# ace19-dev/gvcnn-tf

Measured on AMD Instinct MI355X. Metric: views/sec, higher is better.
Workload: dtype f32; 1 GPU; BASELINE.json configs[1]: ModelNet-shaped, 12 views x 224x224x3, inception_v3 backbone (raw tap Mixed_6e, final tap Mixed_7c), num_groups=7, f32, forward only; views_per_gpu=384, global_views=384, num_groups=7, num_classes=10, exchange=none, branch_lanes=3, launch=eager

## Files before the change

### gvcnn-tf_amd/build.py

```python
import os
import subprocess
import sys

HERE = os.path.dirname(os.path.abspath(__file__))
ROOT = os.path.dirname(HERE)
CSRC = os.path.join(HERE, "csrc")
PT = os.environ.get("GV_PHASE_TIMES") == "1"
LIB = os.path.join(HERE, "libgvcnn_hip_pt.so" if PT else "libgvcnn_hip.so")
BUILD = "build_pt" if PT else "build"
SOURCES = ["conv_igemm.hip", "conv_bf16s.hip", "conv_lp.hip", "conv_dma.hip", "conv_ws.hip", "conv_ws_x3.hip", "conv_chain.hip", "pool.hip", "lowp.hip", "grouping.hip", "plan.hip", "train.hip", "train_lp.hip", "wgrad_dma.hip",
           "retrieval.hip", "render.hip", "metric.hip", "scorer_bwd.hip", "png.hip", "explain.hip"]
FLAGS = ["--offload-arch=gfx950", "-O3", "-std=c++17", "-fPIC", "-Wall",
         "-I" + os.path.join(ROOT, "include"), "-I" + CSRC] + (["-DGV_PHASE_TIMES"] if PT else [])


def _stale(target, deps):
    if not os.path.exists(target):
        return True
    t = os.path.getmtime(target)
    return any(os.path.getmtime(d) > t for d in deps)


def build(force=False, verbose=False):
    hipcc = os.environ.get("HIPCC", "/opt/rocm/bin/hipcc")
    headers = [os.path.join(ROOT, "include", "gvcnn_hip.h")] + sorted(
        os.path.join(CSRC, f) for f in os.listdir(CSRC) if f.endswith(".h"))
    objs = []
    procs = []
    os.makedirs(os.path.join(HERE, BUILD), exist_ok=True)
    for s in SOURCES:
        src = os.path.join(CSRC, s)
        obj = os.path.join(HERE, BUILD, s.replace(".hip", ".o"))
        objs.append(obj)
        if force or _stale(obj, [src] + headers):
            cmd = [hipcc] + FLAGS + ["-c", src, "-o", obj]
            if verbose:
                print(" ".join(cmd))
            procs.append((cmd, subprocess.Popen(cmd)))
    for cmd, p in procs:
        if p.wait() != 0:
            raise RuntimeError("hipcc failed: " + " ".join(cmd))
    if force or procs or _stale(LIB, objs):
        cmd = [hipcc, "--offload-arch=gfx950", "-shared", "-fPIC", "-o", LIB] + objs
        if verbose:
            print(" ".join(cmd))
        subprocess.check_call(cmd)
    return LIB


if __name__ == "__main__":
    print(build(force="--force" in sys.argv, verbose=True))
```

### gvcnn-tf_amd/csrc/conv_common.h

```cpp
#pragma once
#include <cstdlib>

#include "gv_common.h"
#include "conv_stats.h"

namespace gvconv {

struct ConvArgs {
    const float* x;
    const void* w;
    const float* scale;
    const float* shift;
    const float* res;
    float* y;
    float* y2;
    const float* scale2;
    const float* shift2;
    int nb, ih, iw, cin, x_ld;
    int kh, kw, stride, pad_t, pad_l;
    int oh, ow, cout, y_ld, res_ld, y2_ld;
    int M, K, Kpad, ktiles;
    int relu, relu2, split;
    int relu_limit;
    int tiles_n;
    int dil_shift;
#ifdef GV_PHASE_TIMES
    unsigned long long* phase_buf = nullptr;
#endif
    int dbg;
    const void* zeros;
    int y_p3, y2_p3;
    int korder;
    const float* xscale;
    const float* xshift;
    ConvStats st;
    int y_step = 0;
    int y_py = 0, y_px = 0;
    int y_ih = 0, y_iw = 0;
    GvFastDiv y_div_img = {0, -1, 1}, y_div_row = {0, -1, 1};
    int pool = 0;
    int ph = 0, pw = 0;
};

inline bool lp_epilogue_lean_ok(const ConvArgs& a) {
    const bool one = a.y2 == nullptr && a.split == 0;
    const bool two = a.y2 != nullptr && a.split > 0 && a.split % 8 == 0 && a.y2_ld % 8 == 0 && (((uintptr_t)a.y2) & 15) == 0 &&
                     !a.y2_p3;
    return !(a.dbg & 2) && (one || two) && a.cout % 8 == 0 && a.y_ld % 8 == 0 &&
           (((uintptr_t)a.y) & 15) == 0 && (a.res == nullptr || (a.res_ld % 8 == 0 && (((uintptr_t)a.res) & 15) == 0)) &&
           (!a.relu || a.relu_limit >= a.cout || a.relu_limit % 8 == 0);
}

template <int TM, int TN>
__device__ __forceinline__ void conv_epilogue(const ConvArgs& a, const f32x16 (&acc)[TM][TN], int m0,
                                              int n0, int wm, int wn, int lane) {
    if (a.dbg & 4) {
        float t = 0.f;
#pragma unroll
        for (int i = 0; i < TM; ++i)
#pragma unroll
            for (int j = 0; j < TN; ++j)
#pragma unroll
                for (int r = 0; r < 16; ++r) t += acc[i][j][r];
        if (t == 1.2345e-30f) a.y[0] = t;
        return;
    }
    const int col_l = lane & 31;
    const int row_h = 4 * (lane >> 5);
#pragma unroll
    for (int j = 0; j < TN; ++j) {
        const int col = n0 + (wn * TN + j) * 32 + col_l;
        if (col >= a.cout) continue;
        const float sc = a.scale[col], sh = a.shift[col];
        const bool to_second = a.split > 0 && col >= a.split;
        const bool dual = a.y2 != nullptr && a.split == 0;
        const bool relu = a.relu && col < a.relu_limit;
        float sc2 = 0.f, sh2 = 0.f;
        if (dual) { sc2 = a.scale2[col]; sh2 = a.shift2[col]; }
        float* ybase = to_second ? a.y2 + (col - a.split) : a.y + col;
        const int yld = to_second ? a.y2_ld : a.y_ld;
#pragma unroll
        for (int i = 0; i < TM; ++i) {
            const int rbase = m0 + (wm * TM + i) * 32 + row_h;
#pragma unroll
            for (int r = 0; r < 16; ++r) {
                const int m = rbase + (r & 3) + 8 * (r >> 2);
                if (m >= a.M) continue;
                float v = acc[i][j][r] * sc + sh;
                if (a.res) v += a.res[(size_t)m * a.res_ld + col];
                if (dual) {
                    float v2 = v * sc2 + sh2;
                    if (a.relu2) v2 = fmaxf(v2, 0.f);
                    a.y2[(size_t)m * a.y2_ld + col] = v2;
                }
                if (relu) v = fmaxf(v, 0.f);
                ybase[(size_t)m * yld] = v;
            }
        }
    }
}

inline int64_t conv_grid(ConvArgs& a, int bm, int bn) {
    a.tiles_n = gv_ceil_div(a.cout, bn);
    const int64_t nwg = (int64_t)gv_ceil_div(a.M, bm) * a.tiles_n;
    return nwg > 0x7fffffff ? -1 : nwg;
}

inline bool ws_disabled() {
    static const bool off = getenv("GV_NO_WS") != nullptr;
    return off;
}

inline int staged_pick_tile(int M, int N) {
    int best = 0, best_bn = 128;
    double best_cost = 1e30;
    const int order[] = {0, 3, 1, 5}, bns[] = {128, 96, 64, 32};
    const double pen[] = {1.00, 1.02, 1.05, 1.20};
    for (int t = 0; t < 4; ++t) {
        const double cost = (double)gv_ceil_div(N, bns[t]) * bns[t] * pen[t];
        if (cost < best_cost) { best_cost = cost; best = order[t]; best_bn = bns[t]; }
    }
    const int64_t blocks = (int64_t)gv_ceil_div(M, 128) * gv_ceil_div(N, best_bn);
    if (blocks < 1024) {
        if (best_bn == 128) best = 4;
        else if (best_bn == 64) best = 2;
    }
    return best;
}


int bf16s_staged_num_cfgs();
int bf16s_staged_launch(int planes, int cfg, const ConvArgs& a, bool generic, hipStream_t st);
int bf16s_special_launch(int planes, const ConvArgs& a, bool generic, hipStream_t st);
bool bf16s_halo_ok(int planes, const ConvArgs& a, bool generic);
bool bf16s_stem_ok(int planes, const ConvArgs& a);
int bf16s_pack_filter(const float* w_hwio, int kh, int kw, int cin, int cout, int planes, void* out,
                      hipStream_t st);
int64_t bf16s_packed_bytes(int kh, int kw, int cin, int cout, int planes);

int lp_staged_num_cfgs();
int lp_staged_launch(int dtype, int cfg, const ConvArgs& a, bool generic, bool xf32, hipStream_t st);
int lp_special_launch(int dtype, const ConvArgs& a, bool generic, bool xf32, hipStream_t st);
bool lp_xpre_cfg_ok(int cfg);
int lp_xpre_pick(int M, int N);
bool lp_halo_ok(const ConvArgs& a, bool generic);
bool lp_stem_ok(const ConvArgs& a, bool xf32);
int lp_pack_filter(const float* w_hwio, int kh, int kw, int cin, int cout, int dtype, void* out, hipStream_t st);
int64_t lp_packed_bytes(int kh, int kw, int cin, int cout);
int lp_pack_filters_batched(const gv_pack_job* jobs_dev, const int* block_job_dev, int nblocks, int dtype, hipStream_t st);

int dma_lp_num_cfgs();
bool dma_lp_ok(const ConvArgs& a, bool generic, bool xf32);
int dma_lp_launch(int dtype, int cfg, const ConvArgs& a, hipStream_t st);
const void* dma_zero_page();
int dma_x3_num_cfgs();
bool dma_x3_ok(const ConvArgs& a);
int dma_x3_launch(int cfg, const ConvArgs& a, hipStream_t st);
bool chain_tail_ok(const ConvArgs& a);
int chain_tail_launch(int dtype, const ConvArgs& a, hipStream_t st);
int ws_lp_num_cfgs();
int ws_lp_launch(int dtype, int cfg, const ConvArgs& a, hipStream_t st);
int ws_x3_num_cfgs();
int ws_x3_launch(int cfg, const ConvArgs& a, hipStream_t st);
int wsg_x3_num_cfgs();
int wsg_x3_launch(int cfg, const ConvArgs& a, hipStream_t st);

}
```

### gvcnn-tf_amd/csrc/conv_ws_x3.hip

```cpp
#include <cstdlib>
#include <type_traits>

#include "conv_common.h"
#include "conv_lp_epi.h"
#include "conv_x3_epi.h"

namespace {

constexpr int X3W_HEAD = 64;
constexpr int X3W_NL = 4;

struct WsX3Args {
    int taps, nchunks, nk;
    int halo_lo;
    int strip_blocks;
    int pad_[3];
};

__device__ __forceinline__ void x3w_dma16(const char* gsrc, char* lds_dst) {
    __builtin_amdgcn_global_load_lds((const __attribute__((address_space(1))) void*)gsrc,
                                     (__attribute__((address_space(3))) void*)lds_dst, 16, 0, 0);
}
template <int N>
__device__ __forceinline__ void x3w_wait_vm() {
    static_assert(N >= 0 && N < 64, "vmcnt is a 6-bit counter");
    asm volatile("s_waitcnt vmcnt(%0)" ::"n"(N) : "memory");
}

__device__ __forceinline__ void x3w_gload16(f32x4& dst, const char* p) {
    asm volatile("global_load_dwordx4 %0, %1, off" : "=v"(dst) : "v"(p) : "memory");
}
template <int N>
__device__ __forceinline__ void x3w_wait_vm_reg(f32x4& r) {
    static_assert(N >= 0 && N < 64, "vmcnt is a 6-bit counter");
    asm volatile("s_waitcnt vmcnt(%1)" : "+v"(r) : "n"(N) : "memory");
}

template <int WM, int WN, int TM, int TN, int NB, int SBMAX, int GEMM = 0>
__global__ __launch_bounds__((WM * WN + X3W_NL) * 64, 3) void conv_ws_x3(const ConvArgs a, const WsX3Args w) {
    constexpr int NC = WM * WN;
    constexpr int BM = WM * TM * 32, BN = WN * TN * 32;
    constexpr int B_PLANE = BN * 32, B_SLOT = 3 * B_PLANE;
    constexpr int A_PLANE = GEMM ? BM * 32 : X3W_HEAD + SBMAX * 1024, S_BUF = 3 * A_PLANE;
    constexpr int NA = GEMM ? 3 : 2;
    constexpr int OFF_S = NB * B_SLOT;
    constexpr int UB3 = 3 * (BN / 32);
    constexpr int LB = (UB3 + X3W_NL - 1) / X3W_NL;
    static_assert(NC == 8, "eight consumer waves + four loaders: three waves per SIMD");
    static_assert(TM <= TN && TM * TN >= 4, "plane-2 fragments of a and b share one register block");
    static_assert(NB >= 3 && (NB - 1) * LB < 64, "ring depth / vmcnt range");
    static_assert(GEMM == 0 || (NB == 4 && BM % (16 * X3W_NL) == 0), "GEMM mode: four filter slots, 16-row load instructions");
    (void)NA;

    extern __shared__ __attribute__((aligned(128))) char smem[];
    const int tid = threadIdx.x;
    const int lane = tid & 63;
    const int wave = __builtin_amdgcn_readfirstlane(tid >> 6);
    const int lid = gv_xcd_remap(blockIdx.x, gridDim.x);
    const int tile_n = lid % a.tiles_n, tile_m = lid / a.tiles_n;
    const int m0 = tile_m * BM, n0 = tile_n * BN;
    const int nk = w.nk, NTAP = w.taps;
    const bool nosync = (a.dbg & (16384 | 65536)) != 0;

    static_assert(BN <= X3W_NL * 64, "one loader thread per tile column");
    float ss_v[2] = {0.f, 0.f};
    f32x16 acc[TM][TN];

    if (wave >= NC) {
        const int lw = wave - NC;
        if (tid - NC * 64 < BN) {
            const int cc = min(n0 + tid - NC * 64, a.cout - 1);
            ss_v[0] = a.scale[cc];
            ss_v[1] = a.shift[cc];
        }
        if (!(a.dbg & 16384)) {
            __builtin_amdgcn_s_setprio(3);
            const bool nodma = (a.dbg & 32768) != 0, nobar = (a.dbg & 65536) != 0;
            const int lrow = lane >> 1;
            const int lc16 = (((lane & 1) ^ ((lrow >> 3) & 1)) << 4);
            const char* xb = reinterpret_cast<const char*>(a.x);
            const char* b_ptr[LB];
            int b_dst[LB];
            {
                const size_t wrow = (size_t)(a.Kpad / 16) * 96;
#pragma unroll
                for (int i = 0; i < LB; ++i) {
                    int d = lw + i * X3W_NL;
                    d = d < UB3 ? d : UB3 - 1;
                    const int rb = d / 3, p = d - rb * 3;
                    int n = n0 + rb * 32 + lrow;
                    n = n < a.cout ? n : a.cout - 1;
                    b_ptr[i] = reinterpret_cast<const char*>(a.w) + (size_t)n * wrow + p * 32 + lc16;
                    b_dst[i] = p * B_PLANE + rb * 1024;
                }
            }
            int bq_t = 0, bq_c = 0, bq_slot = 0;
            const int gtap = (a.cin >> 4) * 96;
            auto issue_b = [&]() {
                const unsigned koff = (unsigned)(bq_t * gtap + bq_c * 96);
                char* sb = smem + bq_slot * B_SLOT;
#pragma unroll
                for (int i = 0; i < LB; ++i)
                    if (!nodma) x3w_dma16(b_ptr[i] + koff, sb + b_dst[i]);
                if (++bq_t == NTAP) { bq_t = 0; ++bq_c; }
                bq_slot = bq_slot + 1 == NB ? 0 : bq_slot + 1;
            };
            if constexpr (GEMM != 0) {
                constexpr int RPW = BM / X3W_NL, NI = RPW / 16;
                const int qd = lane & 3;
                const char* a_ptr[NI];
                int a_dst[NI];
#pragma unroll
                for (int i = 0; i < NI; ++i) {
                    const int row = lw * RPW + i * 16 + (lane >> 2);
                    int m = m0 + row;
                    m = m < a.M ? m : a.M - 1;
                    a_ptr[i] = xb + (size_t)(unsigned)m * ((size_t)a.x_ld * 4) + qd * 16;
                    a_dst[i] = OFF_S + row * 32 + ((((qd >> 1) ^ ((row >> 3) & 1))) << 4) + (qd & 1) * 8;
                }
                f32x4 stg[2][NI];
                auto load_a = [&](auto sc, int c) {
                    constexpr int S = decltype(sc)::value;
                    c = c < nk ? c : nk - 1;
#pragma unroll
                    for (int i = 0; i < NI; ++i) x3w_gload16(stg[S][i], a_ptr[i] + (size_t)c * 64);
                };
                auto wait_a = [&](auto sc, auto nc) {
                    constexpr int S = decltype(sc)::value;
                    constexpr int N = decltype(nc)::value;
#pragma unroll
                    for (int i = 0; i < NI; ++i) x3w_wait_vm_reg<N>(stg[S][i]);
                };
                auto write_a = [&](auto sc, int slot) {
                    constexpr int S = decltype(sc)::value;
                    char* sb = smem + slot * S_BUF;
#pragma unroll
                    for (int i = 0; i < NI; ++i) {
                        float v[4] = {stg[S][i][0], stg[S][i][1], stg[S][i][2], stg[S][i][3]};
#pragma unroll
                        for (int p = 0; p < 3; ++p) {
                            const unsigned lo = pack2<__bf16>(v[0], v[1]), hi = pack2<__bf16>(v[2], v[3]);
                            typedef unsigned u32x2_t __attribute__((ext_vector_type(2)));
                            *reinterpret_cast<u32x2_t*>(sb + p * A_PLANE + a_dst[i]) = u32x2_t{lo, hi};
                            if (p < 2) {
                                v[0] -= __builtin_bit_cast(float, lo << 16);
                                v[1] -= __builtin_bit_cast(float, lo & 0xffff0000u);
                                v[2] -= __builtin_bit_cast(float, hi << 16);
                                v[3] -= __builtin_bit_cast(float, hi & 0xffff0000u);
                            }
                        }
                    }
                };
                using S0 = std::integral_constant<int, 0>;
                using S1 = std::integral_constant<int, 1>;
                auto fetch = [&](auto sc, int k) {
                    issue_b();
                    load_a(sc, k);
                };
                fetch(S0{}, 0);
                fetch(S1{}, 1);
                wait_a(S0{}, std::integral_constant<int, 0>{});
                wait_a(S1{}, std::integral_constant<int, 0>{});
                write_a(S0{}, 0);
                write_a(S1{}, 1);
                fetch(S0{}, 2);
                fetch(S1{}, 3);
                asm volatile("s_waitcnt lgkmcnt(0)" ::: "memory");
                if (!nobar) __builtin_amdgcn_s_barrier();
                auto iter = [&](auto sc, int j) {
                    wait_a(sc, std::integral_constant<int, LB + NI>{});
                    if (j + 2 < nk) {
                        int slot = j + 2;
                        slot -= (slot / 3) * 3;
                        write_a(sc, slot);
                        asm volatile("s_waitcnt lgkmcnt(0)" ::: "memory");
                    }
                    if (!nobar) __builtin_amdgcn_s_barrier();
                    if (j + 4 >= nk) {
                        bq_c = nk - 1;
                        bq_slot = (nk - 1) & 3;
                    }
                    fetch(sc, j + 4);
                };
                for (int j = 0; j + 1 < nk; j += 2) {
                    iter(S0{}, j);
                    if (j + 2 < nk) iter(S1{}, j + 1);
                }
                x3w_wait_vm<0>();
            } else {
            const unsigned pix_bytes = (unsigned)a.x_ld * 6u;
            int sq_c = 0, sq_buf = 0;
            int sp_blk = 1 << 30, sp_p = 0, sp_c = 0, sp_buf = 0;
            auto strip_begin = [&]() {
                sp_blk = lw / 3; sp_p = lw - sp_blk * 3; sp_c = sq_c; sp_buf = sq_buf;
                ++sq_c;
                sq_buf ^= 1;
            };
            auto strip_units = [&](int n) {
                char* sb = smem + OFF_S + sp_buf * S_BUF + X3W_HEAD;
                const unsigned coff = (unsigned)sp_c * 96u + (unsigned)lc16;
                for (int i = 0; i < n && sp_blk < w.strip_blocks; ++i) {
                    int p = m0 - w.halo_lo + sp_blk * 32 + lrow;
                    p = p < 0 ? 0 : (p < a.M ? p : a.M - 1);
                    if (!nodma) x3w_dma16(xb + (size_t)(unsigned)p * pix_bytes + coff + sp_p * 32, sb + sp_p * A_PLANE + sp_blk * 1024);
                    ++sp_p; ++sp_blk;
                    if (sp_p == 3) { sp_p = 0; ++sp_blk; }
                }
            };
            const int upl = (3 * w.strip_blocks + X3W_NL - 1) / X3W_NL;
            const int win = max(NTAP - NB + 2, 1);
            const int ppi = (upl + win - 1) / win;
            strip_begin();
            strip_units(1 << 20);
            issue_b();
#pragma unroll
            for (int q = 1; q < NB; ++q) issue_b();
            x3w_wait_vm<(NB - 2) * LB>();
            if (!nobar) __builtin_amdgcn_s_barrier();
            if (w.nchunks > 1) { strip_begin(); strip_units(ppi); }
            int ft = 0;
            for (int j = 0; j + 1 < nk; ++j) {
                if (j + NB - 1 <= nk - 1) x3w_wait_vm<(NB - 3) * LB>();
                else x3w_wait_vm<0>();
                if (!nobar) __builtin_amdgcn_s_barrier();
                const bool last_tap = ft + 1 == NTAP;
                if (last_tap && sq_c < w.nchunks) strip_begin();
                strip_units(ppi);
                if (j + NB < nk) issue_b();
                ft = last_tap ? 0 : ft + 1;
            }
            x3w_wait_vm<0>();
            }
        }
    } else {
        const int wm = wave / WN, wn = wave % WN;
        const int r = lane & 31, h = lane >> 5;
        if constexpr (GEMM == 0) {
            if (tid < 96) {
                const int img = tid >> 4;
                *reinterpret_cast<unsigned*>(smem + OFF_S + (img / 3) * S_BUF + (img % 3) * A_PLANE + (tid & 15) * 4) = 0u;
            }
        }
#pragma unroll
        for (int i = 0; i < TM; ++i)
#pragma unroll
            for (int j = 0; j < TN; ++j)
#pragma unroll
                for (int q = 0; q < 16; ++q) acc[i][j][q] = 0.f;
        const int rbase0 = wm * TM * 32 + r + w.halo_lo;
        unsigned tapmask[TM];
        if constexpr (GEMM != 0) {
#pragma unroll
            for (int i = 0; i < TM; ++i) tapmask[i] = 0u;
        } else {
            const int ohow = a.oh * a.ow;
#pragma unroll
            for (int i = 0; i < TM; ++i) {
                const int lr = (wm * TM + i) * 32 + r;
                int m = m0 + lr;
                m = m < a.M ? m : a.M - 1;
                const int n = gv_div(m, a.y_div_img);
                const int rem = m - n * ohow;
                const int y = gv_div(rem, a.y_div_row);
                const int x = rem - y * a.ow;
                const int r_lo = max(0, a.pad_t - y), r_hi = min(a.kh, a.ih + a.pad_t - y);
                const int c_lo = max(0, a.pad_l - x), c_hi = min(a.kw, a.iw + a.pad_l - x);
                const unsigned rowbits = c_hi > c_lo ? (1u << c_hi) - (1u << c_lo) : 0u;
                unsigned tm = 0u;
                for (int fr = 0; fr < a.kh; ++fr)
                    if (fr >= r_lo && fr < r_hi) tm |= rowbits << (fr * a.kw);
                tapmask[i] = tm;
            }
        }
        const int h16 = h << 4;
        const int b_lane = (wn * TN * 32 + r) * 32 + ((((r >> 3) & 1) << 4) ^ h16);
        auto a_addr = [&](int i, int off, int tap, int sbase) -> int {
            if constexpr (GEMM != 0) return sbase + ((wm * TM + i) * 32 + r) * 32 + ((((r >> 3) & 1) << 4) ^ h16);
            const int row = rbase0 + i * 32 + off;
            const int ad = sbase + X3W_HEAD + row * 32 + ((((row >> 3) & 1) << 4) ^ h16);
            const int in = -(int)((tapmask[i] >> tap) & 1u);
            return (ad & in) | ((sbase + h16) & ~in);
        };
        auto lds16 = [&](int addr) -> u32x4 { return *reinterpret_cast<const u32x4*>(smem + addr); };
        u32x4 A0[TM], A1[TM], B0[TN], B1[TN], T[TN];
#define X3W_PIN() __builtin_amdgcn_sched_barrier(0)
        auto kstep = [&](auto nextc, int (&aa)[TM], int& bn, bool bar, auto&& next_addr) {
            constexpr bool NEXT = decltype(nextc)::value;
            constexpr int NM = TM * TN;
            X3W_PIN();
#pragma unroll
            for (int m = 0; m < NM; ++m) {
                const int i = m / TN, j = m % TN;
                acc[i][j] = mfma16<__bf16>(A0[i], T[j], acc[i][j]);
                if (i == TM - 1 && j < TM) { T[j] = lds16(aa[j] + 2 * A_PLANE); X3W_PIN(); }
            }
            X3W_PIN();
            next_addr();
#pragma unroll
            for (int m = 0; m < NM; ++m) {
                const int i = m / TN, j = m % TN;
                acc[i][j] = mfma16<__bf16>(A0[i], B1[j], acc[i][j]);
            }
            X3W_PIN();
#pragma unroll
            for (int m = 0; m < NM; ++m) {
                const int i = m / TN, j = m % TN;
                acc[i][j] = mfma16<__bf16>(A0[i], B0[j], acc[i][j]);
                if constexpr (NEXT) {
                    if (i == 0 && j >= TM && j < TN) { T[j] = lds16(bn + j * 1024 + 2 * B_PLANE); X3W_PIN(); }
                    if (j == TN - 1) { A0[i] = lds16(aa[i]); X3W_PIN(); }
                }
            }
            X3W_PIN();
#pragma unroll
            for (int m = 0; m < NM; ++m) {
                const int i = m / TN, j = m % TN;
                acc[i][j] = mfma16<__bf16>(T[i], B0[j], acc[i][j]);
                if constexpr (NEXT) {
                    if (j == TN - 1) { T[i] = lds16(bn + i * 1024 + 2 * B_PLANE); X3W_PIN(); }
                }
            }
            X3W_PIN();
#pragma unroll
            for (int m = 0; m < NM; ++m) {
                const int i = m / TN, j = m % TN;
                acc[i][j] = mfma16<__bf16>(A1[i], B0[j], acc[i][j]);
                if constexpr (NEXT) {
                    if (i == TM - 1) { B0[j] = lds16(bn + j * 1024); X3W_PIN(); }
                }
            }
            X3W_PIN();
#pragma unroll
            for (int m = 0; m < NM; ++m) {
                const int i = m / TN, j = m % TN;
                acc[i][j] = mfma16<__bf16>(A1[i], B1[j], acc[i][j]);
                if constexpr (NEXT) {
                    if (m == 1) {
                        X3W_PIN();
                        if (bar) __builtin_amdgcn_s_barrier();
                        X3W_PIN();
                    }
                    if (j == TN - 1) { A1[i] = lds16(aa[i] + A_PLANE); X3W_PIN(); }
                    if (i == TM - 1) { B1[j] = lds16(bn + j * 1024 + B_PLANE); X3W_PIN(); }
                }
            }
            X3W_PIN();
        };
        int q_fr = 0, q_fs = 0, q_tap = 0;
        int sbuf = 0, bslot = 0;
        int aa[TM];
#pragma unroll
        for (int i = 0; i < TM; ++i) aa[i] = a_addr(i, -(a.pad_t * a.iw + a.pad_l), 0, OFF_S);
        asm volatile("s_waitcnt lgkmcnt(0)" ::: "memory");
        if (!nosync) __builtin_amdgcn_s_barrier();
#pragma unroll
        for (int i = 0; i < TM; ++i) { A0[i] = lds16(aa[i]); A1[i] = lds16(aa[i] + A_PLANE); }
#pragma unroll
        for (int j = 0; j < TN; ++j) {
            B0[j] = lds16(b_lane + j * 1024);
            B1[j] = lds16(b_lane + j * 1024 + B_PLANE);
            T[j] = lds16(b_lane + j * 1024 + 2 * B_PLANE);
        }
        int bn = 0;
        auto next_addr = [&]() {
            if constexpr (GEMM != 0) {
                sbuf = sbuf + 1 == NA ? 0 : sbuf + 1;
#pragma unroll
                for (int i = 0; i < TM; ++i) aa[i] = a_addr(i, 0, 0, OFF_S + sbuf * S_BUF);
                bslot = bslot + B_SLOT == NB * B_SLOT ? 0 : bslot + B_SLOT;
                bn = b_lane + bslot;
                return;
            }
            const bool wrap = q_tap + 1 == NTAP;
            const bool row_end = q_fs + 1 == a.kw;
            q_tap = wrap ? 0 : q_tap + 1;
            q_fr = wrap ? 0 : (row_end ? q_fr + 1 : q_fr);
            q_fs = (wrap || row_end) ? 0 : q_fs + 1;
            sbuf = wrap ? sbuf ^ 1 : sbuf;
            const int sbase = OFF_S + sbuf * S_BUF;
            const int off = (q_fr - a.pad_t) * a.iw + (q_fs - a.pad_l);
#pragma unroll
            for (int i = 0; i < TM; ++i) aa[i] = a_addr(i, off, q_tap, sbase);
            bslot = bslot + B_SLOT == NB * B_SLOT ? 0 : bslot + B_SLOT;
            bn = b_lane + bslot;
        };
        for (int j = 0; j + 1 < nk; ++j) {
            kstep(std::true_type{}, aa, bn, !nosync, next_addr);
        }
        kstep(std::false_type{}, aa, bn, false, [] {});
#undef X3W_PIN
    }
    __syncthreads();
    constexpr int SS_OFF = NC * X3EpiGeom<TN>::BYTES;
    float* sstab = reinterpret_cast<float*>(smem + SS_OFF);
    if (tid >= NC * 64 && tid - NC * 64 < BN) {
        sstab[tid - NC * 64] = ss_v[0];
        sstab[BN + tid - NC * 64] = ss_v[1];
    }
    __syncthreads();
    if (wave < NC) {
        const int wm = wave / WN, wn = wave % WN;
        x3_epilogue_staged<TM, TN>(a, acc, m0, n0, wm, wn, lane, reinterpret_cast<float*>(smem + wave * X3EpiGeom<TN>::BYTES), sstab, BN);
    }
}

#ifndef GV_KERNEL_ONLY
bool ws_x3_epi_ok(const ConvArgs& a) {
    if (a.cout % 8 != 0 || (a.y2 != nullptr && a.split == 0)) return false;
    if (a.res != nullptr && (a.res_ld % 4 != 0 || !gv_aligned16(a.res))) return false;
    if (!a.y_p3 && (a.y_ld % 4 != 0 || !gv_aligned16(a.y))) return false;
    if (a.split > 0 && (a.split % 8 != 0 || (!a.y2_p3 && (a.y2_ld % 4 != 0 || !gv_aligned16(a.y2))))) return false;
    return true;
}

bool ws_x3_shape_ok(const ConvArgs& a) {
    return a.stride == 1 && a.dil_shift == 0 && a.oh == a.ih && a.ow == a.iw && a.cin % 16 == 0 && a.x_ld % 16 == 0 &&
           a.kh * a.kw <= 32 && a.kw < 32 && a.pad_t < a.kh && a.pad_l < a.kw && a.pool == 0 && a.xscale == nullptr &&
           a.y_step == 0 && a.st.mode == gvconv::STAT_OFF && ws_x3_epi_ok(a);
}

template <int WM, int WN, int TM, int TN, int NB, int SBMAX>
int launch_ws_x3(const ConvArgs& a0, hipStream_t st) {
    constexpr int NC = WM * WN, BM = WM * TM * 32, BN = WN * TN * 32;
    if (!ws_x3_shape_ok(a0)) return GV_E_UNSUPPORTED;
    ConvArgs a = a0;
    a.Kpad = a.K;
    WsX3Args w;
    w.taps = a.kh * a.kw;
    w.nchunks = a.cin / 16;
    w.nk = w.taps * w.nchunks;
    if (w.nk < NB || w.taps < NB - 1) return GV_E_UNSUPPORTED;
    w.halo_lo = a.pad_t * a.iw + a.pad_l;
    const int halo_hi = (a.kh - 1 - a.pad_t) * a.iw + (a.kw - 1 - a.pad_l);
    w.strip_blocks = gv_ceil_div(w.halo_lo + BM + halo_hi, 32);
    if (w.strip_blocks > SBMAX) return GV_E_UNSUPPORTED;
    w.pad_[0] = w.pad_[1] = w.pad_[2] = 0;
    const int64_t nwg = gvconv::conv_grid(a, BM, BN);
    if (nwg < 0) return GV_E_UNSUPPORTED;
    constexpr size_t ring = (size_t)NB * 96 * BN + 6 * (size_t)(X3W_HEAD + SBMAX * 1024);
    constexpr size_t epi = (size_t)NC * X3EpiGeom<TN>::BYTES + 2 * BN * sizeof(float);
    constexpr size_t lds = ring > epi ? ring : epi;
    static_assert(lds <= 160 * 1024, "one workgroup per CU");
    return gv_launch<conv_ws_x3<WM, WN, TM, TN, NB, SBMAX, 0>>(dim3((unsigned)nwg), dim3((NC + X3W_NL) * 64), lds, st, a, w);
}

template <int WM, int WN, int TM, int TN, int MODE>
int launch_wsg_x3(const ConvArgs& a0, hipStream_t st) {
    constexpr int NC = WM * WN, BM = WM * TM * 32, BN = WN * TN * 32, NB = 4;
    const ConvArgs& c = a0;
    if (!(c.kh == 1 && c.kw == 1 && c.stride == 1 && c.pad_t == 0 && c.pad_l == 0 && c.dil_shift == 0 && c.oh == c.ih &&
          c.ow == c.iw && c.cin % 16 == 0 && c.x_ld % 4 == 0 && gv_aligned16(c.x) && c.pool == 0 && c.xscale == nullptr &&
          c.y_step == 0 && c.st.mode == gvconv::STAT_OFF && ws_x3_epi_ok(c)))
        return GV_E_UNSUPPORTED;
    ConvArgs a = a0;
    a.Kpad = a.K;
    WsX3Args w;
    w.taps = 1;
    w.nchunks = a.cin / 16;
    w.nk = w.nchunks;
    if (w.nk < 4) return GV_E_UNSUPPORTED;
    w.halo_lo = 0;
    w.strip_blocks = 0;
    w.pad_[0] = w.pad_[1] = w.pad_[2] = 0;
    const int64_t nwg = gvconv::conv_grid(a, BM, BN);
    if (nwg < 0) return GV_E_UNSUPPORTED;
    constexpr size_t ring = (size_t)NB * 96 * BN + 9 * (size_t)BM * 32;
    constexpr size_t epi = (size_t)NC * X3EpiGeom<TN>::BYTES + 2 * BN * sizeof(float);
    constexpr size_t lds = ring > epi ? ring : epi;
    static_assert(lds <= 160 * 1024, "one workgroup per CU");
    return gv_launch<conv_ws_x3<WM, WN, TM, TN, NB, 0, MODE>>(dim3((unsigned)nwg), dim3((NC + X3W_NL) * 64), lds, st, a, w);
}
#endif

}

#ifndef GV_KERNEL_ONLY
namespace gvconv {

int ws_x3_num_cfgs() { return 5; }

int ws_x3_launch(int cfg, const ConvArgs& a, hipStream_t st) {
    if (ws_disabled()) return GV_E_UNSUPPORTED;
    switch (cfg) {
        case 0: return launch_ws_x3<4, 2, 2, 3, 4, 13>(a, st);
        case 1: return launch_ws_x3<4, 2, 2, 2, 4, 13>(a, st);
        case 2: return launch_ws_x3<8, 1, 2, 3, 3, 21>(a, st);
        case 3: return launch_ws_x3<8, 1, 2, 2, 3, 21>(a, st);
        case 4: return launch_ws_x3<8, 1, 1, 5, 4, 13>(a, st);
    }
    return GV_E_UNSUPPORTED;
}

int wsg_x3_num_cfgs() { return 2; }

int wsg_x3_launch(int cfg, const ConvArgs& a, hipStream_t st) {
    if (ws_disabled()) return GV_E_UNSUPPORTED;
    switch (cfg) {
        case 0: return launch_wsg_x3<4, 2, 2, 3, 1>(a, st);
        case 1: return launch_wsg_x3<4, 2, 2, 2, 1>(a, st);
    }
    return GV_E_UNSUPPORTED;
}

}
#endif
```

Baseline: 30730 views/s.

## Add full-width row-strip kernel for small 1x1 bf16x3 convolutions

Adds a new 1x1 convolution kernel in which each workgroup owns a 128-row strip and covers every output channel (up to 256), so activations are read once and converted to a three-way bf16 split in registers. Weights are streamed into an LDS ring by DMA. The kernel uses smaller workgroups sized so two to four can share a CU, which raises occupancy for the moderate-channel 1x1 layers in Inception. The wsg_x3 configs 0 and 1 now route to this kernel whenever the shape qualifies, with a debug bit to turn it off. The risk is lower per-workgroup MFMA density and fewer workgroups in total for some shapes.

```diff
diff --git a/gvcnn-tf_amd/build.py b/gvcnn-tf_amd/build.py
--- a/gvcnn-tf_amd/build.py
+++ b/gvcnn-tf_amd/build.py
@@ -8,7 +8,7 @@
 PT = os.environ.get("GV_PHASE_TIMES") == "1"
 LIB = os.path.join(HERE, "libgvcnn_hip_pt.so" if PT else "libgvcnn_hip.so")
 BUILD = "build_pt" if PT else "build"
-SOURCES = ["conv_igemm.hip", "conv_bf16s.hip", "conv_lp.hip", "conv_dma.hip", "conv_ws.hip", "conv_ws_x3.hip", "conv_chain.hip", "pool.hip", "lowp.hip", "grouping.hip", "plan.hip", "train.hip", "train_lp.hip", "wgrad_dma.hip",
+SOURCES = ["conv_igemm.hip", "conv_bf16s.hip", "conv_lp.hip", "conv_dma.hip", "conv_ws.hip", "conv_ws_x3.hip", "conv_ws_x3_rows.hip", "conv_chain.hip", "pool.hip", "lowp.hip", "grouping.hip", "plan.hip", "train.hip", "train_lp.hip", "wgrad_dma.hip",
            "retrieval.hip", "render.hip", "metric.hip", "scorer_bwd.hip", "png.hip", "explain.hip"]
 FLAGS = ["--offload-arch=gfx950", "-O3", "-std=c++17", "-fPIC", "-Wall",
          "-I" + os.path.join(ROOT, "include"), "-I" + CSRC] + (["-DGV_PHASE_TIMES"] if PT else [])
diff --git a/gvcnn-tf_amd/csrc/conv_common.h b/gvcnn-tf_amd/csrc/conv_common.h
--- a/gvcnn-tf_amd/csrc/conv_common.h
+++ b/gvcnn-tf_amd/csrc/conv_common.h
@@ -164,5 +164,7 @@
 int ws_x3_launch(int cfg, const ConvArgs& a, hipStream_t st);
 int wsg_x3_num_cfgs();
 int wsg_x3_launch(int cfg, const ConvArgs& a, hipStream_t st);
+bool ws_rows_x3_ok(const ConvArgs& a);
+int ws_rows_x3_launch(const ConvArgs& a, hipStream_t st);
 
 }
diff --git a/gvcnn-tf_amd/csrc/conv_ws_x3.hip b/gvcnn-tf_amd/csrc/conv_ws_x3.hip
--- a/gvcnn-tf_amd/csrc/conv_ws_x3.hip
+++ b/gvcnn-tf_amd/csrc/conv_ws_x3.hip
@@ -444,14 +444,16 @@
     return gv_launch<conv_ws_x3<WM, WN, TM, TN, NB, SBMAX, 0>>(dim3((unsigned)nwg), dim3((NC + X3W_NL) * 64), lds, st, a, w);
 }
 
+bool wsg_x3_shape_ok(const ConvArgs& c) {
+    return c.kh == 1 && c.kw == 1 && c.stride == 1 && c.pad_t == 0 && c.pad_l == 0 && c.dil_shift == 0 && c.oh == c.ih &&
+           c.ow == c.iw && c.cin % 16 == 0 && c.x_ld % 4 == 0 && gv_aligned16(c.x) && c.pool == 0 && c.xscale == nullptr &&
+           c.y_step == 0 && c.st.mode == gvconv::STAT_OFF && ws_x3_epi_ok(c);
+}
+
 template <int WM, int WN, int TM, int TN, int MODE>
 int launch_wsg_x3(const ConvArgs& a0, hipStream_t st) {
     constexpr int NC = WM * WN, BM = WM * TM * 32, BN = WN * TN * 32, NB = 4;
-    const ConvArgs& c = a0;
-    if (!(c.kh == 1 && c.kw == 1 && c.stride == 1 && c.pad_t == 0 && c.pad_l == 0 && c.dil_shift == 0 && c.oh == c.ih &&
-          c.ow == c.iw && c.cin % 16 == 0 && c.x_ld % 4 == 0 && gv_aligned16(c.x) && c.pool == 0 && c.xscale == nullptr &&
-          c.y_step == 0 && c.st.mode == gvconv::STAT_OFF && ws_x3_epi_ok(c)))
-        return GV_E_UNSUPPORTED;
+    if (!wsg_x3_shape_ok(a0)) return GV_E_UNSUPPORTED;
     ConvArgs a = a0;
     a.Kpad = a.K;
     WsX3Args w;
@@ -495,6 +497,7 @@
 
 int wsg_x3_launch(int cfg, const ConvArgs& a, hipStream_t st) {
     if (ws_disabled()) return GV_E_UNSUPPORTED;
+    if ((cfg == 0 || cfg == 1) && !(a.dbg & 262144) && wsg_x3_shape_ok(a) && ws_rows_x3_ok(a)) return ws_rows_x3_launch(a, st);
     switch (cfg) {
         case 0: return launch_wsg_x3<4, 2, 2, 3, 1>(a, st);
         case 1: return launch_wsg_x3<4, 2, 2, 2, 1>(a, st);
diff --git a/gvcnn-tf_amd/csrc/conv_ws_x3_rows.hip b/gvcnn-tf_amd/csrc/conv_ws_x3_rows.hip
--- /dev/null
+++ b/gvcnn-tf_amd/csrc/conv_ws_x3_rows.hip
@@ -0,0 +1,198 @@
+#include <type_traits>
+
+#include "conv_common.h"
+#include "conv_lp_epi.h"
+#include "conv_x3_epi.h"
+
+namespace {
+
+constexpr int XR_NW = 4;
+constexpr int XR_DBG_VM0 = 131072;
+
+template <int NBLK> struct RowsGeom {
+    static constexpr int B_PLANE = NBLK * 1024;
+    static constexpr int SLOT = 3 * B_PLANE;
+    static constexpr int NR = 4 * SLOT <= 72 * 1024 ? 4 : 3;
+    static constexpr int UNITS = 3 * NBLK;
+    static constexpr int LB = (UNITS + XR_NW - 1) / XR_NW;
+    static constexpr int DUMP = NR * SLOT;
+    static constexpr int RING = DUMP + 1024;
+    static constexpr int EPI = XR_NW * X3EpiGeom<NBLK>::BYTES + 2 * NBLK * 32 * (int)sizeof(float);
+    static constexpr int LDS = RING > EPI ? RING : EPI;
+    static constexpr int WGS = NBLK <= 3 ? 4 : 2;
+    static_assert(LDS <= 80 * 1024, "two workgroups per CU");
+    static_assert(WGS * LDS <= 160 * 1024, "the CU's LDS");
+};
+
+__device__ __forceinline__ void xr_dma16(const char* gsrc, unsigned lds_addr) {
+    asm volatile("s_mov_b32 m0, %1\n\ts_nop 0\n\tglobal_load_lds_dwordx4 %0, off" ::"v"(gsrc), "s"(lds_addr) : "memory", "m0");
+}
+__device__ __forceinline__ void xr_gload16(f32x4& dst, const char* p) {
+    asm volatile("global_load_dwordx4 %0, %1, off" : "=v"(dst) : "v"(p) : "memory");
+}
+template <int N>
+__device__ __forceinline__ void xr_wait_vm_reg(f32x4& r) {
+    static_assert(N >= 0 && N < 64, "vmcnt is a 6-bit counter");
+    asm volatile("s_waitcnt vmcnt(%1)" : "+v"(r) : "n"(N) : "memory");
+}
+
+template <typename F, int... Cs>
+__device__ __forceinline__ void xr_for_each(F&& f, std::integer_sequence<int, Cs...>) {
+    (f(std::integral_constant<int, Cs>{}), ...);
+}
+
+template <int NBLK>
+__global__ __launch_bounds__(XR_NW * 64, RowsGeom<NBLK>::WGS) void conv_ws_x3_rows(const ConvArgs a, const int nk) {
+    using G = RowsGeom<NBLK>;
+    constexpr int NR = G::NR, PF = NR - 1, LB = G::LB, SLOT = G::SLOT, B_PLANE = G::B_PLANE;
+    constexpr int GOPS = LB + 2;
+    static_assert((PF - 1) * GOPS < 64, "vmcnt range");
+    extern __shared__ __attribute__((aligned(128))) char smem[];
+    const int tid = threadIdx.x;
+    const int lane = tid & 63;
+    const int wave = __builtin_amdgcn_readfirstlane(tid >> 6);
+    const int m0 = blockIdx.x * (XR_NW * 32);
+    const int r = lane & 31, h = lane >> 5;
+
+    float ss_v[2] = {0.f, 0.f};
+    if (tid < NBLK * 32) {
+        const int cc = min(tid, a.cout - 1);
+        ss_v[0] = a.scale[cc];
+        ss_v[1] = a.shift[cc];
+    }
+    const char* ap;
+    {
+        int m = m0 + wave * 32 + r;
+        m = m < a.M ? m : a.M - 1;
+        ap = reinterpret_cast<const char*>(a.x) + (size_t)(unsigned)m * ((size_t)a.x_ld * 4) + h * 32;
+    }
+    const char* b_ptr[LB];
+    int b_dst[LB];
+    {
+        const int lrow = lane >> 1;
+        const int lc16 = (((lane & 1) ^ ((lrow >> 3) & 1)) << 4);
+        const size_t wrow = (size_t)(a.Kpad / 16) * 96;
+#pragma unroll
+        for (int i = 0; i < LB; ++i) {
+            const int d = wave + i * XR_NW;
+            const int dd = d < G::UNITS ? d : G::UNITS - 1;
+            const int rb = dd / 3, p = dd - rb * 3;
+            int n = rb * 32 + lrow;
+            n = n < a.cout ? n : a.cout - 1;
+            b_ptr[i] = reinterpret_cast<const char*>(a.w) + (size_t)n * wrow + p * 32 + lc16;
+            b_dst[i] = d < G::UNITS ? p * B_PLANE + rb * 1024 : -1;
+        }
+    }
+    const unsigned lds0 = (unsigned)(size_t)((__attribute__((address_space(3))) char*)smem);
+    int ws = 0;
+    f32x4 stg[PF][2];
+    auto fetch = [&](auto sc, int q) {
+        constexpr int S = decltype(sc)::value;
+        const bool live = q < nk;
+        const int qq = live ? q : nk - 1;
+#pragma unroll
+        for (int i = 0; i < LB; ++i) {
+            const int dst = (live && b_dst[i] >= 0) ? ws + b_dst[i] : G::DUMP;
+            xr_dma16(b_ptr[i] + (unsigned)qq * 96u, __builtin_amdgcn_readfirstlane(lds0 + (unsigned)dst));
+        }
+        ws = ws + SLOT == NR * SLOT ? 0 : ws + SLOT;
+        xr_gload16(stg[S][0], ap + (size_t)qq * 64);
+        xr_gload16(stg[S][1], ap + (size_t)qq * 64 + 16);
+    };
+    f32x16 acc[1][NBLK];
+#pragma unroll
+    for (int j = 0; j < NBLK; ++j)
+#pragma unroll
+        for (int q = 0; q < 16; ++q) acc[0][j][q] = 0.f;
+    const bool vm0 = (a.dbg & XR_DBG_VM0) != 0;
+    const int b_lane = r * 32 + ((((r >> 3) & 1) << 4) ^ (h << 4));
+    auto lds16 = [&](int addr) -> u32x4 { return *reinterpret_cast<const u32x4*>(smem + addr); };
+    int rs = 0;
+
+    xr_for_each([&](auto qc) { fetch(qc, decltype(qc)::value); }, std::make_integer_sequence<int, PF>{});
+
+    auto chunk = [&](auto sc, int c) {
+        constexpr int S = decltype(sc)::value;
+        if (vm0) asm volatile("s_waitcnt vmcnt(0)" ::: "memory");
+        xr_wait_vm_reg<(PF - 1) * GOPS>(stg[S][0]);
+        xr_wait_vm_reg<(PF - 1) * GOPS>(stg[S][1]);
+        float v[8] = {stg[S][0][0], stg[S][0][1], stg[S][0][2], stg[S][0][3], stg[S][1][0], stg[S][1][1], stg[S][1][2], stg[S][1][3]};
+        u32x4 A[3];
+#pragma unroll
+        for (int p = 0; p < 3; ++p) {
+#pragma unroll
+            for (int q = 0; q < 4; ++q) {
+                const unsigned d = pack2<__bf16>(v[2 * q], v[2 * q + 1]);
+                A[p][q] = d;
+                if (p < 2) {
+                    v[2 * q] -= __builtin_bit_cast(float, d << 16);
+                    v[2 * q + 1] -= __builtin_bit_cast(float, d & 0xffff0000u);
+                }
+            }
+        }
+        asm volatile("s_waitcnt lgkmcnt(0)" ::: "memory");
+        __builtin_amdgcn_s_barrier();
+        fetch(sc, c + PF);
+        const int sb = rs + b_lane;
+#pragma unroll
+        for (int j = 0; j < NBLK; ++j) {
+            const u32x4 B0 = lds16(sb + j * 1024), B1 = lds16(sb + j * 1024 + B_PLANE), B2 = lds16(sb + j * 1024 + 2 * B_PLANE);
+            acc[0][j] = mfma16<__bf16>(A[0], B2, acc[0][j]);
+            acc[0][j] = mfma16<__bf16>(A[0], B1, acc[0][j]);
+            acc[0][j] = mfma16<__bf16>(A[0], B0, acc[0][j]);
+            acc[0][j] = mfma16<__bf16>(A[2], B0, acc[0][j]);
+            acc[0][j] = mfma16<__bf16>(A[1], B0, acc[0][j]);
+            acc[0][j] = mfma16<__bf16>(A[1], B1, acc[0][j]);
+        }
+        rs = rs + SLOT == NR * SLOT ? 0 : rs + SLOT;
+    };
+    for (int c = 0; c < nk; c += PF) {
+        xr_for_each([&](auto qc) { if (c + decltype(qc)::value < nk) chunk(qc, c + decltype(qc)::value); },
+                    std::make_integer_sequence<int, PF>{});
+    }
+    asm volatile("s_waitcnt vmcnt(0) lgkmcnt(0)" ::: "memory");
+    __syncthreads();
+    float* sstab = reinterpret_cast<float*>(smem + XR_NW * X3EpiGeom<NBLK>::BYTES);
+    if (tid < NBLK * 32) {
+        sstab[tid] = ss_v[0];
+        sstab[NBLK * 32 + tid] = ss_v[1];
+    }
+    __syncthreads();
+    x3_epilogue_staged<1, NBLK>(a, acc, m0, 0, wave, 0, lane, reinterpret_cast<float*>(smem + wave * X3EpiGeom<NBLK>::BYTES), sstab,
+                                NBLK * 32);
+}
+
+template <int NBLK>
+int launch_rows(const ConvArgs& a, int nk, hipStream_t st) {
+    const int64_t nwg = gv_ceil_div(a.M, XR_NW * 32);
+    return gv_launch<conv_ws_x3_rows<NBLK>>(dim3((unsigned)nwg), dim3(XR_NW * 64), RowsGeom<NBLK>::LDS, st, a, nk);
+}
+
+}
+
+namespace gvconv {
+
+bool ws_rows_x3_ok(const ConvArgs& a) {
+    return a.cin % 16 == 0 && a.cin >= 64 && a.cin <= 288 && a.cout % 8 == 0 && a.cout <= 256;
+}
+
+int ws_rows_x3_launch(const ConvArgs& a0, hipStream_t st) {
+    if (!ws_rows_x3_ok(a0)) return GV_E_UNSUPPORTED;
+    ConvArgs a = a0;
+    a.Kpad = a.K;
+    a.tiles_n = 1;
+    const int nk = a.cin / 16;
+    switch (gv_ceil_div(a.cout, 32)) {
+        case 1: return launch_rows<1>(a, nk, st);
+        case 2: return launch_rows<2>(a, nk, st);
+        case 3: return launch_rows<3>(a, nk, st);
+        case 4: return launch_rows<4>(a, nk, st);
+        case 5: return launch_rows<5>(a, nk, st);
+        case 6: return launch_rows<6>(a, nk, st);
+        case 7: return launch_rows<7>(a, nk, st);
+        case 8: return launch_rows<8>(a, nk, st);
+    }
+    return GV_E_UNSUPPORTED;
+}
+
+}
```

Result: no change. 30830 views/s (median of 6 runs) (+0.4%).
